# xcyan/neurips18_hierchical_image_manipulation

Hardware: AMD Instinct MI355X
Metric: mask2image train images/sec at 512x256 bs=8 (higher is better)
Workload: dtype f32; 1 GPU; C2: mask2image Cityscapes-shaped 512x256, GlobalGenerator ngf64/4down/9blocks (182.6M params) + 3-scale PatchGAN + VGG19 loss (synthetic weights), full train step G+D Adam, fp32; global_batch=8, per_gpu_batch=8, parallelism=dp1

## Files before the change

include/him.h:

```cpp
#ifndef HIM_H_
#define HIM_H_

#include <stddef.h>
#include <stdint.h>

#ifdef __cplusplus
extern "C" {
#endif

#define HIM_OK 0
#define HIM_E_INVALID (-1)
#define HIM_E_WORKSPACE (-2)
#define HIM_E_LAUNCH (-3)
#define HIM_E_UNSUPPORTED (-4)

#define HIM_ACT_NONE 0
#define HIM_ACT_RELU 1
#define HIM_ACT_LRELU 2
#define HIM_ACT_TANH 3
#define HIM_ACT_SIGMOID 4

#define HIM_PAD_ZERO 0
#define HIM_PAD_REFLECT 1

const char* him_version(void);
const char* him_arch(void);
const char* him_last_error(void);

#define HIM_TILE_DEFAULT 0
#define HIM_TILE_128x128 1
#define HIM_TILE_128x128_8W 2
#define HIM_TILE_128x256 3
#define HIM_TILE_64x128 4
#define HIM_TILE_64x64 5
#define HIM_TILE_MIXED 6
#define HIM_TILE_128x64 7

#define HIM_ALGO_NO_SPLITK (1u << 0)
#define HIM_ALGO_NO_DFOLD (1u << 1)
#define HIM_ALGO_WINO_PADDED_DGRAD (1u << 2)
#define HIM_ALGO_NO_SMALL_WIN (1u << 3)
#define HIM_ALGO_NO_FEWOUT_TILED (1u << 4)
#define HIM_ALGO_NO_FEWIN_TILED (1u << 5)
#define HIM_ALGO_NO_FEWCH_MFMA (1u << 6)
#define HIM_ALGO_GENERIC_CONV (1u << 7)
#define HIM_ALGO_NO_RESBLOCK_FUSED (1u << 8)
#define HIM_ALGO_NO_BGEMM (1u << 10)
#define HIM_ALGO_NO_ONEHOT_RLE (1u << 11)
#define HIM_ALGO_NO_FEWIN_FOLD (1u << 12)
#define HIM_ALGO_NO_FEWIN_REFLECT (1u << 14)
#define HIM_ALGO_NO_WINO_FUSED2 (1u << 15)
#define HIM_ALGO_NO_BGEMM_PERSISTENT (1u << 16)
#define HIM_ALGO_WINO4_TRAIN_FWD (1u << 13)
#define HIM_ALGO_FROZEN_WEIGHTS (1u << 9)

typedef struct HimAlgo {
  int wino_min_c;
  int wino_fused_min_c;
  int wino_fused_max_c;
  int wino4_min_c;
  int ksplit_max;
  int tile_wb, tile_nb;
  int wino_tblock;
  int wgrad_splits;
  unsigned disable;
  int wino_fused_chunk;
  int wgrad_tile;
} HimAlgo;
void him_algo_resolve(const HimAlgo* in, HimAlgo* out);
void him_algo_from_env(HimAlgo* a);

typedef struct HimConv2d {
  int B, Cin, H, W;
  int Cout, KH, KW;
  int stride, pad;
  int pad_mode;
  int OH, OW;
  int act;
  float slope;
  HimAlgo algo;
} HimConv2d;

size_t him_conv2d_fwd_ws(const HimConv2d* d);
int him_conv2d_fwd(const HimConv2d* d, const float* x, const float* w, const float* bias, float* y, void* ws,
                   size_t ws_bytes, void* stream);
size_t him_conv2d_bwd_data_ws(const HimConv2d* d);
// ... 344 lines not shown
```

neurips18_hierchical_image_manipulation_amd/_cabi.py:

```python
import ctypes as C
import os

_HERE = os.path.dirname(os.path.abspath(__file__))
LIB_PATH = os.path.join(_HERE, 'lib', 'libhim_hip.so')

c_float_p = C.c_void_p
c_int, c_size_t, c_float, c_void_p, c_double = C.c_int, C.c_size_t, C.c_float, C.c_void_p, C.c_double


class HimAlgo(C.Structure):
    _fields_ = [(n, c_int) for n in ('wino_min_c', 'wino_fused_min_c', 'wino_fused_max_c', 'wino4_min_c', 'ksplit_max',
                                     'tile_wb', 'tile_nb', 'wino_tblock', 'wgrad_splits')] + \
               [('disable', C.c_uint), ('wino_fused_chunk', c_int), ('wgrad_tile', c_int)]

    def as_dict(self):
        return {n: int(getattr(self, n)) for n, _ in self._fields_ if n != 'reserved'}


ALGO_NO_SPLITK, ALGO_NO_DFOLD, ALGO_WINO_PADDED_DGRAD, ALGO_NO_SMALL_WIN, ALGO_NO_FEWOUT_TILED, ALGO_NO_FEWIN_TILED, \
    ALGO_NO_FEWCH_MFMA, ALGO_GENERIC_CONV, ALGO_NO_RESBLOCK_FUSED, ALGO_FROZEN_WEIGHTS, ALGO_NO_BGEMM, ALGO_NO_ONEHOT_RLE = (1 << i for i in range(12))
ALGO_NO_FEWIN_FOLD = 1 << 12
ALGO_WINO4_TRAIN_FWD = 1 << 13
ALGO_NO_FEWIN_REFLECT = 1 << 14
ALGO_NO_WINO_FUSED2 = 1 << 15
ALGO_NO_BGEMM_PERSISTENT = 1 << 16
ONEHOT_PART_IDS, ONEHOT_PART_DENSE = 1, 2
TILE_DEFAULT, TILE_128x128, TILE_128x128_8W, TILE_128x256, TILE_64x128, TILE_64x64, TILE_MIXED, TILE_128x64 = range(8)


class HimConv2d(C.Structure):
    _fields_ = [(n, c_int) for n in ('B', 'Cin', 'H', 'W', 'Cout', 'KH', 'KW', 'stride', 'pad', 'pad_mode',
                                     'OH', 'OW', 'act')] + [('slope', c_float), ('algo', HimAlgo)]


class HimDeconv2d(C.Structure):
    _fields_ = [(n, c_int) for n in ('B', 'Cin', 'H', 'W', 'Cout', 'KH', 'KW', 'stride', 'pad', 'out_pad',
                                     'OH', 'OW', 'act')] + [('slope', c_float), ('algo', HimAlgo)]


class HimResBlock(C.Structure):
    _fields_ = [(n, c_int) for n in ('B', 'C', 'H', 'W')] + [('eps', c_float), ('algo', HimAlgo)]


ACT_NONE, ACT_RELU, ACT_LRELU, ACT_TANH, ACT_SIGMOID = 0, 1, 2, 3, 4
PAD_ZERO, PAD_REFLECT = 0, 1

P = c_void_p
_CONV, _DECONV, _RESB, _ALGO = C.POINTER(HimConv2d), C.POINTER(HimDeconv2d), C.POINTER(HimResBlock), C.POINTER(HimAlgo)

_SIGS = {
    'him_version': (C.c_char_p, []),
    'him_arch': (C.c_char_p, []),
    'him_last_error': (C.c_char_p, []),
    'him_conv2d_fwd_ws': (c_size_t, [_CONV]),
    'him_conv2d_fwd': (c_int, [_CONV, P, P, P, P, P, c_size_t, P]),
    'him_conv2d_bwd_data_ws': (c_size_t, [_CONV]),
    'him_conv2d_bwd_data': (c_int, [_CONV, P, P, P, P, c_size_t, P]),
    'him_conv2d_bwd_weight_ws': (c_size_t, [_CONV]),
# ... 215 lines not shown
```

neurips18_hierchical_image_manipulation_amd/csrc/him_conv.hip:

```cpp
#include <stdlib.h>

#include <algorithm>
#include <type_traits>

#include "him_common.h"

namespace him {

#include "him_gconv_fast.inc"
#include "him_wino_fused.inc"
#include "him_wino_fused2.inc"
#include "him_bgemm.inc"

struct WT2Phase {
  float* out;
  int JH, JW;
  long long sh, sw, base;
  long long total;
};
struct WT2P {
  const float* W;
  int M, C2, C2p;
  long long sm, sc;
  WT2Phase ph[4];
// ... 91 lines not shown
      case 47: launch_fewout_tiled<4, 7>(p, st); return true;
    }
  }
#define HIM_SMALL(MMv)                                      \
  case MMv:                                                 \
    if (tj == 7) launch_small_cfg<MMv, 7>(p, maxN, st);      \
    else if (tj == 4) launch_small_cfg<MMv, 4>(p, maxN, st); \
    else if (tj == 3) launch_small_cfg<MMv, 3>(p, maxN, st); \
    else if (tj == 2) launch_small_cfg<MMv, 2>(p, maxN, st); \
    else launch_small_cfg<MMv, 0>(p, maxN, st);              \
    break;
  switch (p.M) {
    HIM_SMALL(1)
    HIM_SMALL(2)
    HIM_SMALL(3)
    HIM_SMALL(4)
  }
#undef HIM_SMALL
  if (p.small_nsplit > 1 && maxN < 256 * 512 && p.C2 >= 64) {
    const long long total = (long long)p.M * maxN;
    hipLaunchKernelGGL(gconv_small_finish_kernel, dim3(std::min<long long>(cdiv(total, 256), 4096)), dim3(256), 0, st, p);
  }
  return true;
}

template <int WM, int WN, int TM, int TN>
static void launch_gconv_cfg(const GConvP& p, dim3 grid, hipStream_t st) {
  if (p.pad_mode == HIM_PAD_REFLECT)
    hipLaunchKernelGGL((gconv_kernel<WM, WN, TM, TN, true>), grid, dim3(256), 0, st, p);
  else
    hipLaunchKernelGGL((gconv_kernel<WM, WN, TM, TN, false>), grid, dim3(256), 0, st, p);
}

static int launch_gconv(const HimAlgo& a, const GConvP& p, hipStream_t st) {
  long long maxN = 0;
  for (int i = 0; i < p.nphase; ++i) {
    long long n = (long long)p.B * p.ph[i].NA * p.ph[i].NC;
    if (n > maxN) maxN = n;
  }
  if (maxN == 0 || p.M <= 0) return HIM_OK;
  if (launch_gconv_small(a, p, maxN, st)) return check_launch("gconv_small");
  if (fewin_tiled_ok(a, p)) {
    launch_fewin_tiled(p, st);
    return check_launch("gconv_fewin_tiled");
  }
  if (p.fast) {
    const unsigned long long img_bytes = (unsigned long long)p.C2 * p.SH * p.SW * 4ull;
    if ((unsigned long long)p.B * img_bytes >= (1ull << 31)) {
      if (p.wbatch || p.ksplit > 1 || img_bytes >= (1ull << 31))
        return fail(HIM_E_UNSUPPORTED, "conv: source tensor of %llu bytes >= 2 GiB cannot be sliced along the batch",
                    (unsigned long long)p.B * img_bytes);
      const int per = (int)(((1ull << 31) - 1) / img_bytes);
      for (int b0 = 0; b0 < p.B; b0 += per) {
        GConvP q = p;
        q.B = std::min(per, p.B - b0);
        q.src = p.src + (size_t)b0 * p.C2 * p.SH * p.SW;
        q.dst = p.dst + (size_t)b0 * p.M * p.DH * p.DW;
        const int rcq = launch_gconv(a, q, st);
        if (rcq) return rcq;
      }
      return HIM_OK;
    }
    const int tile_override = p.atrans ? HIM_TILE_64x128 : (p.wbatch ? a.tile_wb : a.tile_nb);
    const int ks = p.ksplit > 1 ? p.ksplit : 1;
    if (p.M <= 64) {
      dim3 grid(cdiv(maxN, 128) * cdiv(p.M, 64), ks, p.nphase);
      launch_fast_cfg<2, 2, 1, 2>(p, grid, st);
    } else {
      const long long tiles128 = (long long)cdiv(maxN, 128) * cdiv(p.M, 128) * p.nphase;
      const bool big = tile_override == HIM_TILE_128x128 ||
                       (tile_override == HIM_TILE_MIXED && (tiles128 >= 512 || (tiles128 >= 200 && tiles128 <= 256)));
      const long long plane0 = (long long)p.ph[0].NA * p.ph[0].NC;
      const long long tiles256 = (maxN / 256) * cdiv(p.M, 128);
      if (tile_override == HIM_TILE_128x256 && p.wbatch && ks == 1 && p.nphase == 1 && plane0 % 256 == 0 && tiles256 % 512 == 0) {
        dim3 grid((unsigned)tiles256, 1, 1);
        launch_fast_cfg<2, 2, 2, 4>(p, grid, st);
      } else if (tile_override == HIM_TILE_64x64) {
        dim3 grid(cdiv(maxN, 64) * cdiv(p.M, 64), ks, p.nphase);
        launch_fast_cfg<2, 2, 1, 1>(p, grid, st);
      } else if (tile_override == HIM_TILE_128x128_8W) {
        dim3 grid(cdiv(maxN, 128) * cdiv(p.M, 128), ks, p.nphase);
        launch_fast_cfg<2, 4, 2, 1>(p, grid, st);
      } else if (big || (tile_override == HIM_TILE_MIXED && ks > 1)) {
        dim3 grid(cdiv(maxN, 128) * cdiv(p.M, 128), ks, p.nphase);
        launch_fast_cfg<2, 2, 2, 2>(p, grid, st);
      } else if (tile_override == HIM_TILE_128x64 || tile_override == HIM_TILE_MIXED) {
        dim3 grid(cdiv(maxN, 64) * cdiv(p.M, 128), ks, p.nphase);
        launch_fast_cfg<2, 2, 2, 1>(p, grid, st);
      } else {
        dim3 grid(cdiv(maxN, 128) * cdiv(p.M, 64), ks, p.nphase);
        launch_fast_cfg<2, 2, 1, 2>(p, grid, st);
      }
    }
    int rcf = check_launch("gconv_fast");
    if (rcf || ks == 1 || p.kno_finish) return rcf;
    const long long n = (long long)p.B * p.M * p.DH * p.DW;
    hipLaunchKernelGGL(gconv_splitk_finish_kernel, dim3(std::min<long long>(cdiv(n, 256), 8192)), dim3(256), 0, st,
                       (const float*)p.kpart, p.dst, p.bias, n, ks, p.M, p.DH * p.DW, p.act, p.slope);
    return check_launch("gconv_splitk_finish");
  }
  if (p.M <= 32) {
    dim3 grid(cdiv(maxN, 256), cdiv(p.M, 32), p.nphase);
    launch_gconv_cfg<1, 4, 1, 2>(p, grid, st);
  } else if (p.M <= 64) {
    dim3 grid(cdiv(maxN, 128), cdiv(p.M, 64), p.nphase);
    launch_gconv_cfg<1, 4, 2, 1>(p, grid, st);
  } else {
    const long long tiles128 = (long long)cdiv(maxN, 128) * cdiv(p.M, 128) * p.nphase;
    if (tiles128 >= 768) {
      dim3 grid(cdiv(maxN, 128), cdiv(p.M, 128), p.nphase);
      launch_gconv_cfg<2, 2, 2, 2>(p, grid, st);
    } else {
      dim3 grid(cdiv(maxN, 64), cdiv(p.M, 128), p.nphase);
      launch_gconv_cfg<2, 2, 2, 1>(p, grid, st);
    }
  }
  return check_launch("gconv");
}

struct WTransP {
  const float* W;
  float* Wt;
  int Co, Ci, KH, KW, s;
  int nphase;
// ... 169 lines not shown
  P.C2p = K;
  P.K = K;
  P.JH = P.JW = 1;
  P.fJHJW = make_fastdiv(1);
  P.fJW = make_fastdiv(1);
  P.NA = 1;
  P.NC = N;
  return launch_gconv(a, g, st);
}
static int run_wino_conv(const HimAlgo& a, int B, int Csrc, int H, int W, int Mout, int OH, int OW, int po, bool reflect,
                         const float* src, const float* U, const float* bias, int act, float slope, float* dst,
                         float* ws, hipStream_t st, bool fold = false, bool atrans = false, float* keep = nullptr) {
  WinoGeom gi = wino_geom(B, Csrc, H, W, OH, OW, po);
  gi.fold = fold ? 1 : 0;
  float* V = keep ? keep : ws;
  float* Mo = ws + (size_t)16 * Csrc * gi.Tp;
  const int tb = wino_tblock(a);
  const dim3 gin(cdiv(gi.Tp, tb), Csrc);
  if (reflect) hipLaunchKernelGGL((wino_input_kernel<true>), gin, dim3(tb), 0, st, src, V, gi);
  else hipLaunchKernelGGL((wino_input_kernel<false>), gin, dim3(tb), 0, st, src, V, gi);
  int rc = check_launch("wino_input");
  if (rc) return rc;
  rc = wino_batched_gemm(a, U, V, Mo, Mout, Csrc, gi.Tp, st, atrans);
  if (rc) return rc;
  WinoGeom go = gi;
  go.C = Mout;
  hipLaunchKernelGGL(wino_output_kernel, dim3(cdiv(gi.Tp, tb), Mout), dim3(tb), 0, st, (const float*)Mo, dst, bias, go,
                     act, slope);
  return check_launch("wino_output");
}

#include "him_conv_wino4.inc"

#include "him_conv_wgrad.inc"

#include "him_wgrad_fewch.inc"

enum WGradFamily { WGRAD_WINO, WGRAD_HEAD, WGRAD_STEM, WGRAD_SMALL_WIN, WGRAD_SMALL, WGRAD_FAST, WGRAD_GENERIC };
struct WGradShape {
  int M, C, B, H, W, OH, OW, KH, KW, stride, pad, pad_mode;
  int Np() const { return C * KH * KW; }
  int Kdim() const { return B * OH * OW; }
};
static WGradShape wgrad_shape(const HimConv2d* d) {
  return {d->Cout, d->Cin, d->B, d->H, d->W, d->OH, d->OW, d->KH, d->KW, d->stride, d->pad, d->pad_mode};
}
struct WGradPlan {
  HimAlgo algo;
  WGradShape s;
  WGradFamily family;
  int BM, BN;
  int splits;
  int kchunk;
  bool reduce;
  size_t need_bytes;
  size_t slab_bytes;
};
static const int SMALL_WIN_SLOTS = 256;
static int small_wgrad_slices(int C, int Kdim) {
  int s = (2048 + C - 1) / C;
  const int maxs = cdiv(Kdim, 256 * 8);
  if (s > maxs) s = maxs;
  return s < 1 ? 1 : s;
}
static bool small_win_class(int M, int KH, int KW) { return M <= 4 && KH == KW && (KH == 3 || KH == 5 || KH == 7); }
static bool small_class(int M, int KH, int KW) { return M <= 4 && KH == KW && (KH == 7 || KH == 4 || KH == 3); }
static bool wgrad_same_geom(const WGradShape& s) {
  return s.stride == 1 && s.pad == s.KH / 2 && s.OH == s.H && s.OW == s.W && s.H > s.pad && s.W > s.pad;
}
static size_t round256(size_t n) { return (n + 255) / 256 * 256; }

static WGradPlan plan_wgrad(const HimAlgo& a, const WGradShape& s, bool allow_wino) {
  WGradPlan p;
  memset(&p, 0, sizeof(p));
  p.algo = a;
  p.s = s;
  p.splits = 1;
  p.reduce = true;
  const int M = s.M, C = s.C, Kdim = s.Kdim();
  const auto slabs = [&](int n) { return (size_t)n * M * s.Np() * sizeof(float); };
  const bool head_c = fewch_class(a, M, C, s.KH, s.KW), stem_c = fewch_class(a, C, M, s.KH, s.KW);
  const bool win_c = small_win_class(M, s.KH, s.KW), small_c = small_class(M, s.KH, s.KW), fast_c = wgrad_fast_class(a, M, C);
  const int fewch_tc = head_c ? C : M, slices = small_wgrad_slices(C, Kdim), tiny_n = std::max(slices, SMALL_WIN_SLOTS);
  int gBM, gBN, fBM = 0, fBN = 0, fs = 0;
  wgrad_tile(M, &gBM, &gBN);
  int gs = wgrad_splits(M, s.Np(), Kdim, gBM, gBN);
  if (win_c && !small_c && !head_c) gs = std::min(gs, tiny_n);
  if (fast_c) wgrad_fast_cfg(a, M, C, Kdim, s.KH * s.KW, &fBM, &fBN, &fs);
  const size_t generic = gs > 1 ? slabs(gs) : 0, tiny = slabs(tiny_n);
  const bool fits31 = (unsigned long long)s.B * M * s.OH * s.OW * 4ull < (1ull << 31) &&
                      (unsigned long long)s.B * C * s.H * s.W * 4ull < (1ull << 31);
  if (allow_wino && wino_wgrad_ok(a, M, C, s.KH, s.KW, s.stride, s.pad, s.H, s.W) && s.OH == s.H && s.OW == s.W) {
    p.family = WGRAD_WINO;
    p.need_bytes = wino_wgrad_floats(s.B, M, C, s.OH, s.OW) * sizeof(float);
    p.slab_bytes = round256(p.need_bytes);
    return p;
  }
  if ((head_c || stem_c) && wgrad_same_geom(s)) {
    p.family = head_c ? WGRAD_HEAD : WGRAD_STEM;
    p.splits = std::min(fewch_geom(head_c, s.B, s.H, s.W, s.pad).ntask, FEWCH_WGS);
    p.need_bytes = fewch_need_bytes(fewch_tc, s.KH, p.splits);
  } else if (win_c && !algo_off(a, HIM_ALGO_NO_SMALL_WIN) && wgrad_same_geom(s)) {
    p.family = WGRAD_SMALL_WIN;
    p.splits = std::min(s.B * cdiv(s.W, 64) * cdiv(s.H, 64), SMALL_WIN_SLOTS);
    p.need_bytes = slabs(p.splits);
  } else if (small_c) {
    p.family = WGRAD_SMALL;
    p.splits = slices;
    p.kchunk = cdiv(Kdim, slices);
    p.need_bytes = slabs(slices);
  } else if (fast_c && s.OH * s.OW >= 4 && fits31) {
    p.family = WGRAD_FAST;
    p.BM = fBM, p.BN = fBN, p.splits = fs;
    p.kchunk = (cdiv(Kdim, fs) + 31) / 32 * 32;
    p.need_bytes = slabs(fs);
  } else {
    p.family = WGRAD_GENERIC;
    p.BM = gBM, p.BN = gBN, p.splits = gs;
    p.kchunk = (cdiv(Kdim, gs) + 31) / 32 * 32;
    p.reduce = gs > 1;
    p.need_bytes = generic;
  }
  size_t b;
  if (head_c || stem_c) b = std::max(std::max(fewch_need_bytes(fewch_tc, s.KH, FEWCH_WGS), generic), (win_c || small_c) ? tiny : 0);
  else if (win_c || small_c) b = tiny;
  else if (fast_c) b = std::max(slabs(fs), generic);
  else b = generic;
// ... 32 lines not shown
  p.accumulate = pl.family == WGRAD_GENERIC ? accumulate : 0;
  p.fKK = make_fastdiv((uint32_t)(KH * s.KW));
  p.fKW = make_fastdiv((uint32_t)s.KW);
  p.fOW = make_fastdiv((uint32_t)s.OW);
  const dim3 block(256);
  switch (pl.family) {
    case WGRAD_WINO: {
      const WinoGeom gx = wino_geom(B, C, H, W, s.OH, s.OW, 1);
      WinoGeom gd = gx;
      gd.C = M;
      float* Vt = (float*)ws;
      float* dM = Vt + (size_t)16 * C * gx.Tp;
      float* dU = dM + (size_t)16 * M * gx.Tp;
      const int tb = wino_tblock(pl.algo);
      int rcw;
      if (kept_v) {
        hipLaunchKernelGGL(wino_dy_kernel, dim3(cdiv(gx.Tp, tb), M), dim3(tb), 0, st, dy, dM, gd);
        rcw = check_launch("wino_dy");
        if (rcw) return rcw;
        rcw = launch_bgemm(dM, kept_v, dU, M, gx.Tp, C, 16, 4, 0, 0, false, st);
      } else {
        const dim3 gin(cdiv(C, tb), gx.Tp);
        if (refl) hipLaunchKernelGGL((wino_input_t_kernel<true>), gin, dim3(tb), 0, st, x, Vt, gx);
        else hipLaunchKernelGGL((wino_input_t_kernel<false>), gin, dim3(tb), 0, st, x, Vt, gx);
        hipLaunchKernelGGL(wino_dy_kernel, dim3(cdiv(gx.Tp, tb), M), dim3(tb), 0, st, dy, dM, gd);
        rcw = check_launch("wino_wgrad_transforms");
        if (rcw) return rcw;
        rcw = wino_batched_gemm(pl.algo, dM, Vt, dU, M, gx.Tp, C, st);
      }
      if (rcw) return rcw;
      hipLaunchKernelGGL(wino_wgrad_out_kernel, dim3(cdiv(C, 256), M), dim3(256), 0, st, (const float*)dU, dw, M, C,
                         accumulate);
      return check_launch("wino_wgrad_out");
    }
    case WGRAD_HEAD:
    case WGRAD_STEM:
      return run_wgrad_fewch(pl.family == WGRAD_HEAD, dy, x, dw, M, C, B, H, W, KH, s.pad, s.pad_mode, pl.splits, accumulate, ws, st);
    case WGRAD_SMALL_WIN: {
      const int nsx = cdiv(W, 64), rows_per = 64, nyc = cdiv(H, rows_per), ntasks = B * nsx * nyc;
      const dim3 grid(pl.splits, cdiv(C, 4));
#define HIM_SWK(MMv, KSv)                                                                                         \
  if (M == MMv && KH == KSv) {                                                                                    \
    constexpr int TRv = (MMv * KSv * KSv > 90) ? (KSv + 1) / 2 : KSv;   \
    const dim3 gridz(grid.x, grid.y, cdiv(KSv, TRv));                                                             \
    if (refl) hipLaunchKernelGGL((wgrad_small_win_kernel<MMv, KSv, TRv, true>), gridz, block, 0, st, p, nsx, nyc, rows_per, ntasks); \
    else hipLaunchKernelGGL((wgrad_small_win_kernel<MMv, KSv, TRv, false>), gridz, block, 0, st, p, nsx, nyc, rows_per, ntasks);     \
  }
      HIM_SWK(1, 3) HIM_SWK(2, 3) HIM_SWK(3, 3) HIM_SWK(4, 3)
      HIM_SWK(1, 5) HIM_SWK(2, 5) HIM_SWK(3, 5) HIM_SWK(4, 5)
      HIM_SWK(1, 7) HIM_SWK(2, 7) HIM_SWK(3, 7) HIM_SWK(4, 7)
#undef HIM_SWK
      return wgrad_finish(pl, "wgrad_small_win", (const float*)ws, dw, accumulate, st);
    }
    case WGRAD_SMALL: {
      const dim3 grid(C, pl.splits);
#define HIM_WS(MMv, TJv)                                                                             \
  if (M == MMv && KH == TJv) {                                                                       \
    if (refl) hipLaunchKernelGGL((wgrad_small_kernel<MMv, TJv, true>), grid, block, 0, st, p);        \
    else hipLaunchKernelGGL((wgrad_small_kernel<MMv, TJv, false>), grid, block, 0, st, p);            \
  }
      HIM_WS(1, 7) HIM_WS(2, 7) HIM_WS(3, 7) HIM_WS(4, 7)
      HIM_WS(1, 4) HIM_WS(2, 4) HIM_WS(3, 4) HIM_WS(4, 4)
      HIM_WS(1, 3) HIM_WS(2, 3) HIM_WS(3, 3) HIM_WS(4, 3)
#undef HIM_WS
      return wgrad_finish(pl, "wgrad_small", (const float*)ws, dw, accumulate, st);
    }
// ... 563 lines not shown
  r.ksplit_max = algo_off(a, HIM_ALGO_NO_SPLITK) ? 1 : algo_ksplit_max(a);
  r.tile_wb = a.tile_wb == HIM_TILE_DEFAULT ? HIM_TILE_64x128 : a.tile_wb;
  r.tile_nb = a.tile_nb == HIM_TILE_DEFAULT ? HIM_TILE_64x128 : a.tile_nb;
  r.wino_tblock = algo_tblock(a);
  r.wino_fused_chunk = algo_wino_fused_chunk(a);
  r.wgrad_tile = (a.wgrad_tile == 1 || a.wgrad_tile == 2) ? a.wgrad_tile : 0;
  *out = r;
}

void him_algo_from_env(HimAlgo* a) {
  if (!a) return;
  memset(a, 0, sizeof(*a));
  auto geti = [](const char* k, int dflt) { const char* e = getenv(k); return e ? atoi(e) : dflt; };
  a->wino_min_c = getenv("HIM_NO_WINOGRAD") ? -1 : geti("HIM_WINO_MIN_C", 0);
  a->wino_fused_min_c = getenv("HIM_NO_WINO_FUSED") ? -1 : geti("HIM_WINO_FUSED_MIN_C", 0);
  a->wino_fused_max_c = geti("HIM_WINO_FUSED_MAX_C", 0);
  a->wino4_min_c = getenv("HIM_NO_WINO4") ? -1 : geti("HIM_WINO4_MIN_C", 0);
  a->ksplit_max = geti("HIM_KSPLIT_MAX", 0);
  const int tile_all = geti("HIM_GCONV_TILE", 0);
  a->tile_wb = geti("HIM_GCONV_TILE_WB", tile_all);
  a->tile_nb = geti("HIM_GCONV_TILE_NB", tile_all);
  a->wino_tblock = geti("HIM_WINO_TBLOCK", 0);
  a->wgrad_splits = geti("HIM_WGRAD_SPLITS", 0);
  a->wino_fused_chunk = geti("HIM_WINO_FUSED_CHUNK", 0);
  a->wgrad_tile = geti("HIM_WGRAD_TILE", 0);
  const struct { const char* k; unsigned bit; } flags[] = {
      {"HIM_NO_SPLITK", HIM_ALGO_NO_SPLITK},           {"HIM_NO_DFOLD", HIM_ALGO_NO_DFOLD},
      {"HIM_WINO_PADDED_DGRAD", HIM_ALGO_WINO_PADDED_DGRAD}, {"HIM_NO_SMALL_WIN", HIM_ALGO_NO_SMALL_WIN},
      {"HIM_NO_FEWOUT_TILED", HIM_ALGO_NO_FEWOUT_TILED}, {"HIM_NO_FEWIN_TILED", HIM_ALGO_NO_FEWIN_TILED},
      {"HIM_NO_FEWCH_MFMA", HIM_ALGO_NO_FEWCH_MFMA},   {"HIM_GENERIC_CONV", HIM_ALGO_GENERIC_CONV},
      {"HIM_NO_RESBLOCK_FUSED", HIM_ALGO_NO_RESBLOCK_FUSED}, {"HIM_NO_BGEMM", HIM_ALGO_NO_BGEMM},
      {"HIM_NO_ONEHOT_RLE", HIM_ALGO_NO_ONEHOT_RLE},   {"HIM_NO_FEWIN_FOLD", HIM_ALGO_NO_FEWIN_FOLD},
      {"HIM_WINO4_TRAIN_FWD", HIM_ALGO_WINO4_TRAIN_FWD}, {"HIM_NO_FEWIN_REFLECT", HIM_ALGO_NO_FEWIN_REFLECT},
      {"HIM_NO_WINO_FUSED2", HIM_ALGO_NO_WINO_FUSED2}, {"HIM_NO_BGEMM_PERSISTENT", HIM_ALGO_NO_BGEMM_PERSISTENT}};
  for (const auto& f : flags)
    if (getenv(f.k)) a->disable |= f.bit;
}

int him_winograd_gemm(const float* a, const float* b, float* c, int M, int K, int N, const HimAlgo* algo, void* stream) {
  if (!a || !b || !c || M <= 4 || K < 16 || (K % 16) || N <= 0 || (N % 128))
    return fail(HIM_E_INVALID, "winograd gemm: need M > 4, K %% 16 == 0, N %% 128 == 0 (got %d, %d, %d)", M, K, N);
  if ((long long)16 * K * N >= (1ll << 31) || (long long)16 * M * N >= (1ll << 31))
    return fail(HIM_E_UNSUPPORTED, "winograd gemm: operand larger than 2^31 elements");
  HimAlgo z;
  memset(&z, 0, sizeof(z));
  return wino_batched_gemm(algo ? *algo : z, a, b, c, M, K, N, (hipStream_t)stream);
}

size_t him_conv2d_fwd_ws(const HimConv2d* d) { return d ? plan_fprop(d).ws_bytes : 0; }

int him_conv2d_fwd(const HimConv2d* d, const float* x, const float* w, const float* bias, float* y, void* ws,
                   size_t ws_bytes, void* stream) {
  int rc = check_conv(d);
  if (rc) return rc;
  return run_fprop(d, x, w, bias, y, ws, ws_bytes, (hipStream_t)stream);
}

int him_conv2d_in_act_fused(const HimConv2d* d) { return (d && !check_conv(d) && plan_fprop(d).in_act_slab) ? 1 : 0; }

int him_conv2d_in_act_fwd(const HimConv2d* d, const float* x, const float* w, const void* panel, const float* bias,
                          float* y_raw, const float* residual, float* z, float* mean, float* rstd, float eps, int act,
                          float slope, void* ws, size_t ws_bytes, void* stream) {
  int rc = check_conv(d);
  if (rc) return rc;
  if (d->act != HIM_ACT_NONE) return fail(HIM_E_INVALID, "conv_in_act: the activation follows the norm (descriptor act must be none)");
  if (!y_raw || !z || !mean || !rstd) return fail(HIM_E_INVALID, "conv_in_act: null output");
  if (panel && !plan_fprop(d).panel_floats) return fail(HIM_E_INVALID, "conv_in_act: no panel for this descriptor");
  hipStream_t st = (hipStream_t)stream;
  FpropDefer df;
// ... 402 lines not shown
```

neurips18_hierchical_image_manipulation_amd/csrc/him_gconv_fast.inc:

```
typedef float f32x16 __attribute__((ext_vector_type(16)));
#define PAD_DFOLD 2
typedef const __attribute__((address_space(1))) char* gchar_p;
typedef const __attribute__((address_space(1))) float* gfloat_p;

struct GPhase {
  const float* A;
  int K;
  int JH, JW;
  FastDiv fJHJW, fJW;
  int NA, NC;
  int oy0, ox0;
  int offy, offx;
  const float* At;
  int C2p;
};

struct GConvP {
  const float* src;
  float* dst;
  const float* bias;
  int M, C2, B, SH, SW, DH, DW;
  int oys, oxs, sy, sx, dy, dx;
  int pad_mode, act;
  float slope;
// ... 235 lines not shown

  const int act = p.act;
  const float slope = p.slope;
  const bool partial = ksplit > 1;
  float* __restrict__ dstbase = partial ? p.kpart + (size_t)blockIdx.y * p.B * p.M * p.DH * p.DW : p.dst;
#pragma unroll
  for (int j = 0; j < TN; ++j) {
    const int nn = n0 + wn * TN * 32 + j * 32 + l31;
    if (nn >= Ntot) continue;
    const int bb = nn / plane;
    const int r2 = nn - bb * plane;
    const int aa = r2 / ph.NC, cc = r2 - aa * ph.NC;
    const int oy = ph.oy0 + p.oys * aa, ox = ph.ox0 + p.oxs * cc;
    float* __restrict__ out = dstbase + ((size_t)bb * p.M * p.DH + oy) * p.DW + ox;
    const size_t mstride = (size_t)p.DH * p.DW;
#pragma unroll
    for (int i = 0; i < TM; ++i) {
#pragma unroll
      for (int r = 0; r < 16; ++r) {
        const int m = m0 + wm * TM * 32 + i * 32 + (r & 3) + 8 * (r >> 2) + 4 * lh;
        if (m < p.M) {
          float v = acc[i][j][r];
          if (!partial) {
            if (p.bias) v += p.bias[m];
            v = apply_act(v, act, slope);
          }
          out[(size_t)m * mstride] = v;
        }
      }
    }
  }
}

__global__ void gconv_splitk_finish_kernel(const float* __restrict__ part, float* __restrict__ dst,
                                           const float* __restrict__ bias, long long n, int ksplit, int M, int plane,
                                           int act, float slope) {
  if ((n & 3) == 0 && (plane & 3) == 0) {
    const float4* __restrict__ p4 = (const float4*)part;
    float4* __restrict__ d4 = (float4*)dst;
    const long long n4 = n >> 2;
    for (long long i = (long long)blockIdx.x * blockDim.x + threadIdx.x; i < n4;
         i += (long long)gridDim.x * blockDim.x) {
      float4 v = p4[i];
      for (int z = 1; z < ksplit; ++z) {
        const float4 w = p4[(size_t)z * n4 + i];
        v.x += w.x; v.y += w.y; v.z += w.z; v.w += w.w;
      }
      const float bb = bias ? bias[(int)(((i << 2) / plane) % M)] : 0.f;
      v.x = apply_act(v.x + bb, act, slope);
      v.y = apply_act(v.y + bb, act, slope);
      v.z = apply_act(v.z + bb, act, slope);
      v.w = apply_act(v.w + bb, act, slope);
      d4[i] = v;
    }
    return;
  }
  for (long long i = (long long)blockIdx.x * blockDim.x + threadIdx.x; i < n;
       i += (long long)gridDim.x * blockDim.x) {
    float v = 0.f;
    for (int z = 0; z < ksplit; ++z) v += part[(size_t)z * n + i];
    if (bias) v += bias[(int)((i / plane) % M)];
    dst[i] = apply_act(v, act, slope);
  }
}

template <int WM, int WN, int TM, int TN>
static void launch_fast_cfg(const GConvP& p, dim3 grid, hipStream_t st) {
  const bool clampc = (p.C2 % 16) != 0;
  const dim3 blk(WM * WN * 64);
  if (p.atrans) {
    if constexpr (WM == 2 && WN == 2 && TM == 1 && TN == 2)
      hipLaunchKernelGGL((gconv_fast_kernel<2, 2, 1, 2, 3, false>), grid, blk, 0, st, p);
    return;
  }
  if (p.pad_mode == PAD_DFOLD) {
    if (clampc) hipLaunchKernelGGL((gconv_fast_kernel<WM, WN, TM, TN, 2, true>), grid, blk, 0, st, p);
    else hipLaunchKernelGGL((gconv_fast_kernel<WM, WN, TM, TN, 2, false>), grid, blk, 0, st, p);
  } else if (p.pad_mode == HIM_PAD_REFLECT) {
    if (clampc) hipLaunchKernelGGL((gconv_fast_kernel<WM, WN, TM, TN, 1, true>), grid, blk, 0, st, p);
    else hipLaunchKernelGGL((gconv_fast_kernel<WM, WN, TM, TN, 1, false>), grid, blk, 0, st, p);
  } else {
    if (clampc) hipLaunchKernelGGL((gconv_fast_kernel<WM, WN, TM, TN, 0, true>), grid, blk, 0, st, p);
    else hipLaunchKernelGGL((gconv_fast_kernel<WM, WN, TM, TN, 0, false>), grid, blk, 0, st, p);
  }
}
```

Baseline: 158.9 images/s.

## Add direct-to-LDS buffer-load pipelined variant of the 64x128 fast gconv kernel

```diff
diff --git a/include/him.h b/include/him.h
--- a/include/him.h
+++ b/include/him.h
@@ -51,6 +51,7 @@
 #define HIM_ALGO_NO_FEWIN_REFLECT (1u << 14)
 #define HIM_ALGO_NO_WINO_FUSED2 (1u << 15)
 #define HIM_ALGO_NO_BGEMM_PERSISTENT (1u << 16)
+#define HIM_OPT_GCONV_DMA (1u << 17)
 #define HIM_ALGO_WINO4_TRAIN_FWD (1u << 13)
 #define HIM_ALGO_FROZEN_WEIGHTS (1u << 9)
 
diff --git a/neurips18_hierchical_image_manipulation_amd/_cabi.py b/neurips18_hierchical_image_manipulation_amd/_cabi.py
--- a/neurips18_hierchical_image_manipulation_amd/_cabi.py
+++ b/neurips18_hierchical_image_manipulation_amd/_cabi.py
@@ -24,6 +24,7 @@
 ALGO_NO_FEWIN_REFLECT = 1 << 14
 ALGO_NO_WINO_FUSED2 = 1 << 15
 ALGO_NO_BGEMM_PERSISTENT = 1 << 16
+OPT_GCONV_DMA = 1 << 17
 ONEHOT_PART_IDS, ONEHOT_PART_DENSE = 1, 2
 TILE_DEFAULT, TILE_128x128, TILE_128x128_8W, TILE_128x256, TILE_64x128, TILE_64x64, TILE_MIXED, TILE_128x64 = range(8)
 
diff --git a/neurips18_hierchical_image_manipulation_amd/csrc/him_conv.hip b/neurips18_hierchical_image_manipulation_amd/csrc/him_conv.hip
--- a/neurips18_hierchical_image_manipulation_amd/csrc/him_conv.hip
+++ b/neurips18_hierchical_image_manipulation_amd/csrc/him_conv.hip
@@ -147,6 +147,14 @@
     hipLaunchKernelGGL((gconv_kernel<WM, WN, TM, TN, false>), grid, dim3(256), 0, st, p);
 }
 
+static bool gconv_dma_ok(const HimAlgo& a, const GConvP& p) {
+  return algo_off(a, HIM_OPT_GCONV_DMA) && !p.atrans && !p.wbatch;
+}
+static void launch_fast_64x128(const HimAlgo& a, const GConvP& p, dim3 grid, hipStream_t st) {
+  if (gconv_dma_ok(a, p)) launch_fast_dma(p, grid, st);
+  else launch_fast_cfg<2, 2, 1, 2>(p, grid, st);
+}
+
 static int launch_gconv(const HimAlgo& a, const GConvP& p, hipStream_t st) {
   long long maxN = 0;
   for (int i = 0; i < p.nphase; ++i) {
@@ -180,7 +188,7 @@
     const int ks = p.ksplit > 1 ? p.ksplit : 1;
     if (p.M <= 64) {
       dim3 grid(cdiv(maxN, 128) * cdiv(p.M, 64), ks, p.nphase);
-      launch_fast_cfg<2, 2, 1, 2>(p, grid, st);
+      launch_fast_64x128(a, p, grid, st);
     } else {
       const long long tiles128 = (long long)cdiv(maxN, 128) * cdiv(p.M, 128) * p.nphase;
       const bool big = tile_override == HIM_TILE_128x128 ||
@@ -204,7 +212,7 @@
         launch_fast_cfg<2, 2, 2, 1>(p, grid, st);
       } else {
         dim3 grid(cdiv(maxN, 128) * cdiv(p.M, 64), ks, p.nphase);
-        launch_fast_cfg<2, 2, 1, 2>(p, grid, st);
+        launch_fast_64x128(a, p, grid, st);
       }
     }
     int rcf = check_launch("gconv_fast");
@@ -1228,7 +1236,8 @@
       {"HIM_NO_RESBLOCK_FUSED", HIM_ALGO_NO_RESBLOCK_FUSED}, {"HIM_NO_BGEMM", HIM_ALGO_NO_BGEMM},
       {"HIM_NO_ONEHOT_RLE", HIM_ALGO_NO_ONEHOT_RLE},   {"HIM_NO_FEWIN_FOLD", HIM_ALGO_NO_FEWIN_FOLD},
       {"HIM_WINO4_TRAIN_FWD", HIM_ALGO_WINO4_TRAIN_FWD}, {"HIM_NO_FEWIN_REFLECT", HIM_ALGO_NO_FEWIN_REFLECT},
-      {"HIM_NO_WINO_FUSED2", HIM_ALGO_NO_WINO_FUSED2}, {"HIM_NO_BGEMM_PERSISTENT", HIM_ALGO_NO_BGEMM_PERSISTENT}};
+      {"HIM_NO_WINO_FUSED2", HIM_ALGO_NO_WINO_FUSED2}, {"HIM_NO_BGEMM_PERSISTENT", HIM_ALGO_NO_BGEMM_PERSISTENT},
+      {"HIM_GCONV_DMA", HIM_OPT_GCONV_DMA}};
   for (const auto& f : flags)
     if (getenv(f.k)) a->disable |= f.bit;
 }
diff --git a/neurips18_hierchical_image_manipulation_amd/csrc/him_gconv_fast.inc b/neurips18_hierchical_image_manipulation_amd/csrc/him_gconv_fast.inc
--- a/neurips18_hierchical_image_manipulation_amd/csrc/him_gconv_fast.inc
+++ b/neurips18_hierchical_image_manipulation_amd/csrc/him_gconv_fast.inc
@@ -291,6 +291,259 @@
   }
 }
 
+#ifndef HIM_GC_DMA_ST
+#define HIM_GC_DMA_ST 3
+#endif
+#ifndef HIM_GC_DMA_PRIO
+#define HIM_GC_DMA_PRIO 1
+#endif
+#ifndef HIM_GC_DMA_DRIP
+#define HIM_GC_DMA_DRIP 1
+#endif
+typedef int i32x4_rsrc __attribute__((ext_vector_type(4)));
+__device__ __forceinline__ void blds4x8(i32x4_rsrc rsrc, unsigned voff, const unsigned (&so)[8], unsigned lds_dst) {
+  unsigned keep;
+  asm volatile(
+      "s_nop 4\n\ts_mov_b32 %0, m0\n\ts_mov_b32 m0, %3\n\ts_nop 0\n\t"
+      "buffer_load_dword %1, %2, %4 offen lds\n\ts_add_u32 m0, m0, 0x200\n\ts_nop 0\n\t"
+      "buffer_load_dword %1, %2, %5 offen lds\n\ts_add_u32 m0, m0, 0x200\n\ts_nop 0\n\t"
+      "buffer_load_dword %1, %2, %6 offen lds\n\ts_add_u32 m0, m0, 0x200\n\ts_nop 0\n\t"
+      "buffer_load_dword %1, %2, %7 offen lds\n\ts_add_u32 m0, m0, 0x200\n\ts_nop 0\n\t"
+      "buffer_load_dword %1, %2, %8 offen lds\n\ts_add_u32 m0, m0, 0x200\n\ts_nop 0\n\t"
+      "buffer_load_dword %1, %2, %9 offen lds\n\ts_add_u32 m0, m0, 0x200\n\ts_nop 0\n\t"
+      "buffer_load_dword %1, %2, %10 offen lds\n\ts_add_u32 m0, m0, 0x200\n\ts_nop 0\n\t"
+      "buffer_load_dword %1, %2, %11 offen lds\n\t"
+      "s_mov_b32 m0, %0"
+      : "=&s"(keep)
+      : "v"(voff), "s"(rsrc), "s"(lds_dst), "s"(so[0]), "s"(so[1]), "s"(so[2]), "s"(so[3]), "s"(so[4]), "s"(so[5]),
+        "s"(so[6]), "s"(so[7])
+      : "memory", "scc");
+}
+
+__device__ __forceinline__ void blds4(i32x4_rsrc rsrc, unsigned voff, unsigned so, unsigned lds_dst) {
+  unsigned keep;
+  asm volatile("s_nop 4\n\ts_mov_b32 %0, m0\n\ts_mov_b32 m0, %3\n\ts_nop 0\n\tbuffer_load_dword %1, %2, %4 offen lds\n\ts_mov_b32 m0, %0"
+               : "=&s"(keep)
+               : "v"(voff), "s"(rsrc), "s"(lds_dst), "s"(so)
+               : "memory");
+}
+
+template <int PM, bool CLAMPC>
+__global__ __launch_bounds__(256, HIM_GC_DMA_ST == 3 ? 4 : 3) void gconv_fast_dma_kernel(const GConvP p) {
+  constexpr int BM = 64, BN = 128, BK = 16, TN = 2, ST = HIM_GC_DMA_ST;
+  constexpr int AF = BM * BK, BF = BK * BN, STF = AF + BF;
+  constexpr int NREQ = 9;
+  static_assert(PM >= 0 && PM <= 2 && ST >= 3 && ST <= 4, "pad modes 0..2, three or four stages");
+  __shared__ __attribute__((aligned(16))) float lds[ST * STF];
+
+  const GPhase& ph = p.ph[blockIdx.z];
+  const int plane = ph.NA * ph.NC;
+  const int Ntot = p.B * plane;
+  int m0, n0;
+  {
+    const int nmt = (p.M + BM - 1) / BM, nnt = gridDim.x / nmt;
+    const int total = nmt * nnt, L = blockIdx.x;
+    const int q = total >> 3, r = total & 7, xcd = L & 7, slot = L >> 3;
+    const int T = (xcd < r ? xcd * (q + 1) : r * (q + 1) + (xcd - r) * q) + slot;
+    if (p.wbatch) {
+      const int ntp = plane / BN, per = nmt * ntp;
+      const int img = T / per, rem = T - img * per;
+      const int mt = rem / ntp;
+      m0 = mt * BM;
+      n0 = img * plane + (rem - mt * ntp) * BN;
+    } else {
+      const int mt = T / nnt;
+      m0 = mt * BM;
+      n0 = (T - mt * nnt) * BN;
+    }
+  }
+  if (n0 >= Ntot) return;
+  const int t = threadIdx.x, lane = t & 63, l31 = lane & 31, lh = lane >> 5;
+  const int wave = __builtin_amdgcn_readfirstlane(t >> 6);
+  const int wn = wave & 1, wm = wave >> 1;
+  const unsigned lds_base = lds_addr_u(lds);
+  const float* __restrict__ At = ph.At + (size_t)(p.wbatch ? n0 / plane : 0) * p.wbatch;
+  const int C2 = p.C2, C2p = ph.C2p, CB = C2p / BK;
+  const int JW = ph.JW, JH = ph.JH;
+  const int nk_all = JH * JW * CB;
+  const uint32_t Kp = (uint32_t)nk_all * BK;
+  const int ksplit = gridDim.y;
+  const int kt0 = (int)(((long long)nk_all * blockIdx.y) / ksplit);
+  const int nk = (int)(((long long)nk_all * (blockIdx.y + 1)) / ksplit) - kt0;
+
+  const int arow = 16 * wave + (lane >> 2);
+  const char* __restrict__ ga = (const char*)At +
+      ((size_t)min(m0 + arow, p.M - 1) * Kp + (size_t)kt0 * BK + (((lane & 3) ^ ((arow >> 2) & 3)) * 4)) * 4;
+
+  const int nl = 64 * wn + lane, kg = wm;
+  const int n = min(n0 + nl, Ntot - 1);
+  const int b = n / plane;
+  const int rr = n - b * plane;
+  const int a = rr / ph.NC;
+  const int c = rr - a * ph.NC;
+  const int by = a * p.sy + ph.offy, bx = c * p.sx + ph.offx;
+  const int SH = p.SH, SW = p.SW;
+  const uint32_t SHSW = (uint32_t)SH * SW;
+  const uint32_t boff = (uint32_t)b * C2 * SHSW;
+  const int ddy = p.dy, ddx = p.dx;
+  const uint32_t chan_bytes = SHSW * 4u;
+  i32x4_rsrc rsrc;
+  {
+    const unsigned long long sp = (unsigned long long)p.src;
+    rsrc.x = __builtin_amdgcn_readfirstlane((int)(unsigned)sp);
+    rsrc.y = __builtin_amdgcn_readfirstlane((int)((unsigned)(sp >> 32) & 0xffffu));
+    rsrc.z = __builtin_amdgcn_readfirstlane((int)((uint32_t)p.B * (uint32_t)C2 * SHSW * 4u));
+    rsrc.w = 0x00020000;
+  }
+  int c_cb = kt0 / (JH * JW);
+  int c_jh = (kt0 - c_cb * JH * JW) / JW;
+  int c_jw = kt0 - c_cb * JH * JW - c_jh * JW;
+  int lk = 0, lslot = 0;
+  const unsigned a_dst = lds_base + (unsigned)(wave * 256 * 4);
+  const unsigned b_dst = lds_base + (unsigned)((AF + 8 * kg * BN + 64 * wn) * 4);
+  uint32_t tapbyte;
+  unsigned so[8], sl;
+#define HIM_GD_ADDR()                                                                                        \
+  {                                                                                                          \
+    int iy = by + c_jh * ddy, ix = bx + c_jw * ddx;                                                          \
+    bool ok = true;                                                                                          \
+    if (PM == 2) {                                                                                           \
+      const int Hh = SH - 2, Ww = SW - 2;  \
+      ok = iy >= 0 && iy < Hh && ix >= 0 && ix < Ww;                                                          \
+      iy = (c_jh == 0 && iy == 2) ? Hh : iy;                                                                 \
+      iy = (c_jh == 2 && iy == Hh - 3) ? Hh + 1 : iy;                                                        \
+      ix = (c_jw == 0 && ix == 2) ? Ww : ix;                                                                 \
+      ix = (c_jw == 2 && ix == Ww - 3) ? Ww + 1 : ix;                                                        \
+    } else if (PM == 1) {                                                                                    \
+      iy = iy < 0 ? -iy : iy;                                                                                \
+      iy = iy >= SH ? 2 * (SH - 1) - iy : iy;                                                                \
+      ix = ix < 0 ? -ix : ix;                                                                                \
+      ix = ix >= SW ? 2 * (SW - 1) - ix : ix;                                                                \
+    } else {                                                                                                 \
+      ok = iy >= 0 && iy < SH && ix >= 0 && ix < SW;                                                          \
+    }                                                                                                        \
+    tapbyte = ok ? (boff + (uint32_t)iy * (uint32_t)SW + (uint32_t)ix) * 4u : 0x80000000u;                    \
+    const int c0 = c_cb * BK + kg * 8;                                                                       \
+    so[0] = (uint32_t)(CLAMPC ? min(c0, C2 - 1) : c0) * chan_bytes;                                           \
+    _Pragma("unroll") for (int i = 0; i < 7; ++i)                                                            \
+        so[i + 1] = so[i] + ((CLAMPC && c0 + i + 1 > C2 - 1) ? 0u : chan_bytes);                              \
+    sl = (unsigned)(lslot * STF * 4);                                                                        \
+  }
+#define HIM_GD_NEXT()                                                                                        \
+  {                                                                                                          \
+    lslot = lslot + 1 == ST ? 0 : lslot + 1;                                                                 \
+    if (lk + 1 < nk) {                   \
+      ++lk;                                                                                                  \
+      ++c_jw;                                                                                                \
+      const bool w1 = c_jw == JW;                                                                            \
+      c_jw = w1 ? 0 : c_jw;                                                                                  \
+      c_jh += w1 ? 1 : 0;                                                                                    \
+      const bool w2 = c_jh == JH;                                                                            \
+      c_jh = w2 ? 0 : c_jh;                                                                                  \
+      c_cb += w2 ? 1 : 0;                                                                                    \
+    }                                                                                                        \
+  }
+#define HIM_GD_LOAD()                                      \
+  {                                                                                                          \
+    HIM_GD_ADDR()                                                                                            \
+    glds16(ga + (size_t)lk * (BK * 4), a_dst + sl);                                                          \
+    blds4x8(rsrc, tapbyte, so, b_dst + sl);                                                                  \
+    HIM_GD_NEXT()                                                                                            \
+  }
+
+  f32x16 acc[TN];
+#pragma unroll
+  for (int j = 0; j < TN; ++j)
+#pragma unroll
+    for (int r = 0; r < 16; ++r) acc[j][r] = 0.f;
+
+  const int ra = wm * 32 + l31;
+  const int aoff0 = ra * BK + (((2 * lh) ^ ((ra >> 2) & 3)) * 4), aoff1 = ra * BK + (((2 * lh + 1) ^ ((ra >> 2) & 3)) * 4);
+  const int boffc = AF + 8 * lh * BN + wn * 64 + l31;
+
+#pragma unroll
+  for (int s = 0; s < ST - 1; ++s) HIM_GD_LOAD()
+  asm volatile("s_waitcnt vmcnt(%0)" ::"n"(NREQ * (ST - 2)) : "memory");
+  __syncthreads();
+  int cslot = 0;
+  for (int kt = 0; kt < nk; ++kt) {
+    const float* __restrict__ sa = lds + cslot * STF;
+#if HIM_GC_DMA_DRIP
+    HIM_GD_ADDR()
+#else
+#if HIM_GC_DMA_PRIO
+    __builtin_amdgcn_s_setprio(3);
+#endif
+    HIM_GD_LOAD()
+#if HIM_GC_DMA_PRIO
+    __builtin_amdgcn_s_setprio(0);
+#endif
+#endif
+    const float4 a0 = *(const float4*)(sa + aoff0), a1 = *(const float4*)(sa + aoff1);
+    float bv[TN][8];
+#pragma unroll
+    for (int j = 0; j < TN; ++j)
+#pragma unroll
+      for (int kp = 0; kp < 8; ++kp) bv[j][kp] = sa[boffc + kp * BN + j * 32];
+    const float av[8] = {a0.x, a0.y, a0.z, a0.w, a1.x, a1.y, a1.z, a1.w};
+#if HIM_GC_DMA_DRIP
+    __builtin_amdgcn_sched_group_barrier(0x100, 10, 0);
+    __builtin_amdgcn_sched_barrier(0);
+#pragma unroll
+    for (int kp = 0; kp < 8; ++kp) {
+#pragma unroll
+      for (int j = 0; j < TN; ++j) acc[j] = __builtin_amdgcn_mfma_f32_32x32x2f32(av[kp], bv[j][kp], acc[j], 0, 0, 0);
+      if (kp == 0) glds16(ga + (size_t)lk * (BK * 4), a_dst + sl);
+      blds4(rsrc, tapbyte, so[kp], b_dst + sl + 512u * kp);
+      __builtin_amdgcn_sched_barrier(0);
+    }
+    HIM_GD_NEXT()
+#else
+#pragma unroll
+    for (int kp = 0; kp < 8; ++kp)
+#pragma unroll
+      for (int j = 0; j < TN; ++j) acc[j] = __builtin_amdgcn_mfma_f32_32x32x2f32(av[kp], bv[j][kp], acc[j], 0, 0, 0);
+    __builtin_amdgcn_sched_group_barrier(0x100, 10, 0);
+    __builtin_amdgcn_sched_group_barrier(0x008, 8 * TN, 0);
+#endif
+    asm volatile("s_waitcnt vmcnt(%0)" ::"n"(NREQ * (ST - 2)) : "memory");
+    __syncthreads();
+    cslot = cslot + 1 == ST ? 0 : cslot + 1;
+  }
+  asm volatile("s_waitcnt vmcnt(0)" ::: "memory");
+#undef HIM_GD_LOAD
+#undef HIM_GD_ADDR
+#undef HIM_GD_NEXT
+
+  const int act = p.act;
+  const float slope = p.slope;
+  const bool partial = ksplit > 1;
+  float* __restrict__ dstbase = partial ? p.kpart + (size_t)blockIdx.y * p.B * p.M * p.DH * p.DW : p.dst;
+#pragma unroll
+  for (int j = 0; j < TN; ++j) {
+    const int nn = n0 + wn * TN * 32 + j * 32 + l31;
+    if (nn >= Ntot) continue;
+    const int bb = nn / plane;
+    const int r2 = nn - bb * plane;
+    const int aa = r2 / ph.NC, cc = r2 - aa * ph.NC;
+    const int oy = ph.oy0 + p.oys * aa, ox = ph.ox0 + p.oxs * cc;
+    float* __restrict__ out = dstbase + ((size_t)bb * p.M * p.DH + oy) * p.DW + ox;
+    const size_t mstride = (size_t)p.DH * p.DW;
+#pragma unroll
+    for (int r = 0; r < 16; ++r) {
+      const int m = m0 + wm * 32 + (r & 3) + 8 * (r >> 2) + 4 * lh;
+      if (m < p.M) {
+        float v = acc[j][r];
+        if (!partial) {
+          if (p.bias) v += p.bias[m];
+          v = apply_act(v, act, slope);
+        }
+        out[(size_t)m * mstride] = v;
+      }
+    }
+  }
+}
+
 __global__ void gconv_splitk_finish_kernel(const float* __restrict__ part, float* __restrict__ dst,
                                            const float* __restrict__ bias, long long n, int ksplit, int M, int plane,
                                            int act, float slope) {
@@ -323,6 +576,21 @@
   }
 }
 
+static void launch_fast_dma(const GConvP& p, dim3 grid, hipStream_t st) {
+  const bool clampc = (p.C2 % 16) != 0;
+  const dim3 blk(256);
+  if (p.pad_mode == PAD_DFOLD) {
+    if (clampc) hipLaunchKernelGGL((gconv_fast_dma_kernel<2, true>), grid, blk, 0, st, p);
+    else hipLaunchKernelGGL((gconv_fast_dma_kernel<2, false>), grid, blk, 0, st, p);
+  } else if (p.pad_mode == HIM_PAD_REFLECT) {
+    if (clampc) hipLaunchKernelGGL((gconv_fast_dma_kernel<1, true>), grid, blk, 0, st, p);
+    else hipLaunchKernelGGL((gconv_fast_dma_kernel<1, false>), grid, blk, 0, st, p);
+  } else {
+    if (clampc) hipLaunchKernelGGL((gconv_fast_dma_kernel<0, true>), grid, blk, 0, st, p);
+    else hipLaunchKernelGGL((gconv_fast_dma_kernel<0, false>), grid, blk, 0, st, p);
+  }
+}
+
 template <int WM, int WN, int TM, int TN>
 static void launch_fast_cfg(const GConvP& p, dim3 grid, hipStream_t st) {
   const bool clampc = (p.C2 % 16) != 0;
```

Result: no change. 158.7 images/s, median of 2 (-0.1%).

## Add polyphase Winograd weight-gradient path for stride-2 3x3 convolutions

Applied to the files above, without the earlier changes.

```diff
diff --git a/include/him.h b/include/him.h
--- a/include/him.h
+++ b/include/him.h
@@ -52,6 +52,7 @@
 #define HIM_ALGO_NO_WINO_FUSED2 (1u << 15)
 #define HIM_ALGO_NO_BGEMM_PERSISTENT (1u << 16)
 #define HIM_ALGO_WINO4_TRAIN_FWD (1u << 13)
+#define HIM_OPT_POLY_WINO (1u << 17)
 #define HIM_ALGO_FROZEN_WEIGHTS (1u << 9)
 
 typedef struct HimAlgo {
diff --git a/neurips18_hierchical_image_manipulation_amd/_cabi.py b/neurips18_hierchical_image_manipulation_amd/_cabi.py
--- a/neurips18_hierchical_image_manipulation_amd/_cabi.py
+++ b/neurips18_hierchical_image_manipulation_amd/_cabi.py
@@ -24,6 +24,7 @@
 ALGO_NO_FEWIN_REFLECT = 1 << 14
 ALGO_NO_WINO_FUSED2 = 1 << 15
 ALGO_NO_BGEMM_PERSISTENT = 1 << 16
+OPT_POLY_WINO = 1 << 17
 ONEHOT_PART_IDS, ONEHOT_PART_DENSE = 1, 2
 TILE_DEFAULT, TILE_128x128, TILE_128x128_8W, TILE_128x256, TILE_64x128, TILE_64x64, TILE_MIXED, TILE_128x64 = range(8)
 
diff --git a/neurips18_hierchical_image_manipulation_amd/csrc/him_conv.hip b/neurips18_hierchical_image_manipulation_amd/csrc/him_conv.hip
--- a/neurips18_hierchical_image_manipulation_amd/csrc/him_conv.hip
+++ b/neurips18_hierchical_image_manipulation_amd/csrc/him_conv.hip
@@ -440,11 +440,13 @@
 
 #include "him_conv_wino4.inc"
 
+#include "him_conv_poly.inc"
+
 #include "him_conv_wgrad.inc"
 
 #include "him_wgrad_fewch.inc"
 
-enum WGradFamily { WGRAD_WINO, WGRAD_HEAD, WGRAD_STEM, WGRAD_SMALL_WIN, WGRAD_SMALL, WGRAD_FAST, WGRAD_GENERIC };
+enum WGradFamily { WGRAD_WINO, WGRAD_HEAD, WGRAD_STEM, WGRAD_SMALL_WIN, WGRAD_SMALL, WGRAD_FAST, WGRAD_GENERIC, WGRAD_POLY };
 struct WGradShape {
   int M, C, B, H, W, OH, OW, KH, KW, stride, pad, pad_mode;
   int Np() const { return C * KH * KW; }
@@ -501,6 +503,13 @@
   if (allow_wino && wino_wgrad_ok(a, M, C, s.KH, s.KW, s.stride, s.pad, s.H, s.W) && s.OH == s.H && s.OW == s.W) {
     p.family = WGRAD_WINO;
     p.need_bytes = wino_wgrad_floats(s.B, M, C, s.OH, s.OW) * sizeof(float);
+    p.slab_bytes = round256(p.need_bytes);
+    return p;
+  }
+  if (poly_wgrad_ok(a, M, C, s.KH, s.KW, s.stride, s.pad, s.pad_mode, s.H, s.W)) {
+    p.family = WGRAD_POLY;
+    p.splits = poly_wgrad_chunks(s.B, M, C, s.OH, s.OW);
+    p.need_bytes = poly_wgrad_floats(s.B, M, C, s.OH, s.OW) * sizeof(float);
     p.slab_bytes = round256(p.need_bytes);
     return p;
   }
@@ -599,6 +608,24 @@
       hipLaunchKernelGGL(wino_wgrad_out_kernel, dim3(cdiv(C, 256), M), dim3(256), 0, st, (const float*)dU, dw, M, C,
                          accumulate);
       return check_launch("wino_wgrad_out");
+    }
+    case WGRAD_POLY: {
+      const PolyGeom gx = poly_geom(B, C, H, W, s.OH, s.OW, pl.splits);
+      PolyGeom gd = gx;
+      gd.C = M;
+      float* V = (float*)ws;
+      float* dM = V + (size_t)25 * C * gx.Tp;
+      float* dU = dM + (size_t)25 * M * gx.Tp;
+      const int tb = wino_tblock(pl.algo);
+      hipLaunchKernelGGL(poly_input_kernel, dim3(cdiv(gx.Tp, tb), C), dim3(tb), 0, st, x, V, gx);
+      hipLaunchKernelGGL(poly_dy_kernel, dim3(cdiv(gx.Tp, tb), M), dim3(tb), 0, st, dy, dM, gd);
+      int rcp = check_launch("poly_wgrad_transforms");
+      if (rcp) return rcp;
+      rcp = launch_bgemm(dM, V, dU, M, gx.Tk, C, 25 * pl.splits, 5, 0, 0, false, st);
+      if (rcp) return rcp;
+      hipLaunchKernelGGL(poly_wgrad_out_kernel, dim3(cdiv(C, 256), M), dim3(256), 0, st, (const float*)dU, dw, M, C, pl.splits,
+                         accumulate);
+      return check_launch("poly_wgrad_out");
     }
     case WGRAD_HEAD:
     case WGRAD_STEM:
@@ -1231,6 +1258,7 @@
       {"HIM_NO_WINO_FUSED2", HIM_ALGO_NO_WINO_FUSED2}, {"HIM_NO_BGEMM_PERSISTENT", HIM_ALGO_NO_BGEMM_PERSISTENT}};
   for (const auto& f : flags)
     if (getenv(f.k)) a->disable |= f.bit;
+  if (!getenv("HIM_NO_POLY_WINO")) a->disable |= HIM_OPT_POLY_WINO;
 }
 
 int him_winograd_gemm(const float* a, const float* b, float* c, int M, int K, int N, const HimAlgo* algo, void* stream) {
diff --git a/neurips18_hierchical_image_manipulation_amd/csrc/him_conv_poly.inc b/neurips18_hierchical_image_manipulation_amd/csrc/him_conv_poly.inc
--- /dev/null
+++ b/neurips18_hierchical_image_manipulation_amd/csrc/him_conv_poly.inc
@@ -0,0 +1,174 @@
+struct PolyGeom {
+  int B, C, H, W;
+  int OH, OW;
+  int TY, TX, T, Tp;
+  int ks, Tk;
+};
+static PolyGeom poly_geom(int B, int C, int H, int W, int OH, int OW, int ks) {
+  PolyGeom g;
+  g.B = B; g.C = C; g.H = H; g.W = W; g.OH = OH; g.OW = OW;
+  g.TY = (OH + 1) / 2; g.TX = (OW + 1) / 2;
+  g.T = B * g.TY * g.TX;
+  g.ks = ks;
+  g.Tp = (g.T + 128 * ks - 1) / (128 * ks) * (128 * ks);
+  g.Tk = g.Tp / ks;
+  return g;
+}
+__device__ __forceinline__ size_t poly_slab_off(const PolyGeom& g, int c, int t) {
+  const int s = t / g.Tk;
+  return ((size_t)s * g.C + c) * g.Tk + (t - s * g.Tk);
+}
+
+__global__ __launch_bounds__(256) void poly_input_kernel(const float* __restrict__ x, float* __restrict__ V,
+                                                         const PolyGeom g) {
+  const int t = blockIdx.x * blockDim.x + threadIdx.x;
+  const int c = blockIdx.y;
+  if (t >= g.Tp) return;
+  float d[5][5];
+  if (t < g.T) {
+    const int per = g.TY * g.TX;
+    const int b = t / per, r = t - b * per, ty = r / g.TX, tx = r - ty * g.TX;
+    const float* __restrict__ src = x + ((size_t)b * g.C + c) * g.H * g.W;
+    int ys[5], xs[5];
+    bool oky[5], okx[5];
+#pragma unroll
+    for (int i = 0; i < 5; ++i) {
+      const int iy = 4 * ty - 1 + i, ix = 4 * tx - 1 + i;
+      const int cy = min(max(iy, 0), g.H - 1), cx = min(max(ix, 0), g.W - 1);
+      oky[i] = cy == iy;
+      okx[i] = cx == ix;
+      ys[i] = cy * g.W;
+      xs[i] = cx;
+    }
+#pragma unroll
+    for (int i = 0; i < 5; ++i)
+#pragma unroll
+      for (int j = 0; j < 5; ++j) {
+        const float v = src[ys[i] + xs[j]];
+        d[i][j] = (oky[i] && okx[j]) ? v : 0.f;
+      }
+  } else {
+#pragma unroll
+    for (int i = 0; i < 5; ++i)
+#pragma unroll
+      for (int j = 0; j < 5; ++j) d[i][j] = 0.f;
+  }
+  float tt[5][5];
+#pragma unroll
+  for (int j = 0; j < 5; ++j) {
+    tt[0][j] = d[1][j];
+    tt[1][j] = d[3][j];
+    tt[2][j] = d[0][j] - d[2][j];
+    tt[3][j] = d[2][j];
+    tt[4][j] = d[4][j] - d[2][j];
+  }
+  const size_t slab = (size_t)g.C * g.Tp;
+  float* __restrict__ o = V + poly_slab_off(g, c, t);
+#pragma unroll
+  for (int i = 0; i < 5; ++i) {
+    o[(size_t)(i * 5 + 0) * slab] = tt[i][1];
+    o[(size_t)(i * 5 + 1) * slab] = tt[i][3];
+    o[(size_t)(i * 5 + 2) * slab] = tt[i][0] - tt[i][2];
+    o[(size_t)(i * 5 + 3) * slab] = tt[i][2];
+    o[(size_t)(i * 5 + 4) * slab] = tt[i][4] - tt[i][2];
+  }
+}
+
+__global__ __launch_bounds__(256) void poly_dy_kernel(const float* __restrict__ dy, float* __restrict__ dM,
+                                                      const PolyGeom g) {
+  const int t = blockIdx.x * blockDim.x + threadIdx.x;
+  const int c = blockIdx.y;
+  if (t >= g.Tp) return;
+  float e[2][2] = {{0.f, 0.f}, {0.f, 0.f}};
+  if (t < g.T) {
+    const int per = g.TY * g.TX;
+    const int b = t / per, rr = t - b * per, ty = rr / g.TX, tx = rr - ty * g.TX;
+    const float* __restrict__ src = dy + ((size_t)b * g.C + c) * g.OH * g.OW;
+#pragma unroll
+    for (int i = 0; i < 2; ++i)
+#pragma unroll
+      for (int j = 0; j < 2; ++j) {
+        const int oy = 2 * ty + i, ox = 2 * tx + j;
+        if (oy < g.OH && ox < g.OW) e[i][j] = src[oy * g.OW + ox];
+      }
+  }
+  float q[5][2];
+#pragma unroll
+  for (int j = 0; j < 2; ++j) {
+    q[0][j] = e[0][j];
+    q[1][j] = e[1][j];
+    q[2][j] = e[0][j];
+    q[3][j] = e[0][j] + e[1][j];
+    q[4][j] = e[1][j];
+  }
+  const size_t slab = (size_t)g.C * g.Tp;
+  float* __restrict__ o = dM + poly_slab_off(g, c, t);
+#pragma unroll
+  for (int i = 0; i < 5; ++i) {
+    o[(size_t)(i * 5 + 0) * slab] = q[i][0];
+    o[(size_t)(i * 5 + 1) * slab] = q[i][1];
+    o[(size_t)(i * 5 + 2) * slab] = q[i][0];
+    o[(size_t)(i * 5 + 3) * slab] = q[i][0] + q[i][1];
+    o[(size_t)(i * 5 + 4) * slab] = q[i][1];
+  }
+}
+
+__global__ __launch_bounds__(256) void poly_wgrad_out_kernel(const float* __restrict__ dU, float* __restrict__ dw,
+                                                             int M, int C, int ks, int accumulate) {
+  __shared__ float so[256 * 9];
+  const int c0 = blockIdx.x * 256, t = threadIdx.x, m = blockIdx.y;
+  const int c = c0 + t;
+  const size_t mc = (size_t)M * C;
+  if (c < C) {
+    const float* __restrict__ in = dU + (size_t)m * C + c;
+    float u[5][5];
+#pragma unroll
+    for (int i = 0; i < 5; ++i)
+#pragma unroll
+      for (int j = 0; j < 5; ++j) {
+        const float* __restrict__ pz = in + (size_t)(i * 5 + j) * ks * mc;
+        float s = pz[0];
+        for (int z = 1; z < ks; ++z) s += pz[(size_t)z * mc];
+        u[i][j] = s;
+      }
+    float e[3][5];
+#pragma unroll
+    for (int j = 0; j < 5; ++j) {
+      e[0][j] = u[2][j] + u[3][j];
+      e[1][j] = u[0][j] + u[1][j];
+      e[2][j] = u[3][j] + u[4][j];
+    }
+#pragma unroll
+    for (int i = 0; i < 3; ++i) {
+      so[t * 9 + i * 3 + 0] = e[i][2] + e[i][3];
+      so[t * 9 + i * 3 + 1] = e[i][0] + e[i][1];
+      so[t * 9 + i * 3 + 2] = e[i][3] + e[i][4];
+    }
+  }
+  __syncthreads();
+  const int nvalid = min(256, C - c0) * 9;
+  float* __restrict__ o = dw + ((size_t)m * C + c0) * 9;
+#pragma unroll
+  for (int k = 0; k < 9; ++k) {
+    const int idx = k * 256 + t;
+    if (idx < nvalid) o[idx] = accumulate ? o[idx] + so[idx] : so[idx];
+  }
+}
+
+static bool poly_wgrad_ok(const HimAlgo& a, int M, int C, int KH, int KW, int stride, int pad, int pad_mode, int H, int W) {
+  return (a.disable & HIM_OPT_POLY_WINO) != 0 && !algo_off(a, HIM_ALGO_NO_BGEMM) && algo_wino_min_c(a) > 0 && KH == 3 &&
+         KW == 3 && stride == 2 && pad == 1 && pad_mode == HIM_PAD_ZERO && (H % 2) == 0 && (W % 2) == 0 && M >= 256 &&
+         C >= 256 && (M % 128) == 0 && (C % 128) == 0;
+}
+static int poly_wgrad_chunks(int B, int M, int C, int OH, int OW) {
+  const int T = B * ((OH + 1) / 2) * ((OW + 1) / 2);
+  const int tiles = 25 * (M / 128) * (C / 128);
+  int ks = 1;
+  while (ks < 8 && tiles * ks < 512 && (T + 2 * ks - 1) / (2 * ks) >= 64) ks *= 2;
+  return ks;
+}
+static size_t poly_wgrad_floats(int B, int M, int C, int OH, int OW) {
+  const int ks = poly_wgrad_chunks(B, M, C, OH, OW);
+  const PolyGeom g = poly_geom(B, C, 1, 1, OH, OW, ks);
+  return (size_t)25 * (C + M) * g.Tp + (size_t)25 * ks * M * C;
+}
```

Result: no change. 160.5 images/s before, 161.6 images/s after, median of 6 (+0.7%).
